# mrjoshuak/go-jpeg2000

Measured on AMD Instinct MI355X. Metric: Mpixels/s encode+decode (4K sRGB, 5-3 lossless), higher is better.
Workload: dtype int32

## Files before the change

go-jpeg2000_amd/csrc/ht.hip:

```cpp
#include <cstdlib>

#include "ht_tables.h"
#include "j2k_internal.h"

namespace j2k {

__device__ __constant__ uint16_t c_vlc_tbl0[1024] = J2K_HT_VLC_TBL0_INIT;
__device__ __constant__ uint16_t c_vlc_tbl1[1024] = J2K_HT_VLC_TBL1_INIT;
__device__ uint16_t g_vlc_enc[2 * 4 * 16];

__global__ void ht_build_enc_table() {
    const int t = threadIdx.x;
    if (t >= 128) return;
    const int initial = t >> 6, context = (t >> 4) & 3, rho = t & 15;
    const uint16_t *tbl = initial ? c_vlc_tbl0 : c_vlc_tbl1;
    uint16_t r = 0x0001;
    for (uint32_t cwd = 0; cwd < 128; cwd++) {
        const uint16_t e = tbl[(context << 7) | cwd];
        if (((e >> 4) & 0xF) == rho && (e & 0xF) > 0) { r = (uint16_t)((cwd << 4) | (e & 0xF)); break; }
    }
    g_vlc_enc[t] = r;
}

__device__ uint16_t g_vlc_pair1[16384];
// ... 1126 lines not shown
                                                         const uint32_t *__restrict__ lens, uint32_t *__restrict__ vbits,
                                                         uint32_t *__restrict__ pairs) {
    __shared__ uint32_t vb4[4][HT_VBITS_WORDS + 8];
    uint32_t *vb = vb4[threadIdx.x >> 6];
    const int jid = blockIdx.x * 4 + (threadIdx.x >> 6);
    if (jid >= njobs) return;
    const int lane = threadIdx.x & 63;
    if (ht_vlcprep_block(jobs, jid, stream, offs, lens, lane, vb, pairs + (size_t)jid * HT_WALK_REC)) return;
    uint32_t *dst = vbits + (size_t)jid * HT_VBITS_WORDS;
    for (int i = lane; i < HT_VBITS_WORDS; i += 64) dst[i] = vb[i];
}

__global__ __launch_bounds__(256) void ht_vlcprep_dedup_kernel(const BlockJob *__restrict__ jobs, int njobs,
                                                               const uint8_t *__restrict__ stream, const uint64_t *__restrict__ offs,
                                                               const uint32_t *__restrict__ lens, uint32_t *__restrict__ vbits,
                                                               uint32_t *__restrict__ pairs, const int32_t *__restrict__ rep) {
    __shared__ uint32_t vb4[4][HT_VBITS_WORDS + 8];
    uint32_t *vb = vb4[threadIdx.x >> 6];
    const int jid = blockIdx.x * 4 + (threadIdx.x >> 6);
    if (jid >= njobs) return;
    const int lane = threadIdx.x & 63;
    uint32_t *rec = pairs + (size_t)jid * HT_WALK_REC;
    const int ldr = rep[jid];
    const uint64_t loff = offs[ldr];
    const uint32_t llen = lens[ldr];
    const HtVlcHead H = ht_vlc_head(jobs, jid, stream, offs, lens);
    const long nb = H.tag ? 0 : ht_vlc_nbytes(H);
    uint32_t pre[HT_VLC_STEPS];
#pragma unroll
    for (int c = 0; c < HT_VLC_STEPS; c++) pre[c] = ht_vlc_load4(H.data, (long)H.len, nb, 1 + 256 * c + 4 * lane);
    if (ldr != jid && H.tag == 0 && llen == H.len && H.len >= 4) {
        const uint8_t *mine = H.data, *theirs = stream + loff;
        const uint32_t len = H.len, nd = (len + 3) >> 2;
        bool same = true;
        for (uint32_t j0 = 0; j0 < nd && same; j0 += 256) {
            uint32_t x[4], y[4];
#pragma unroll
            for (int c = 0; c < 4; c++) {
                const uint32_t p = min(4 * (j0 + 64 * c + lane), len - 4);
                __builtin_memcpy(&x[c], mine + p, 4);
                __builtin_memcpy(&y[c], theirs + p, 4);
            }
            same = __all((x[0] == y[0]) & (x[1] == y[1]) & (x[2] == y[2]) & (x[3] == y[3]));
        }
        if (same) {
            if (lane == 0) { rec[0] = HT_PAIR_DUP; rec[1] = (uint32_t)ldr; rec[HT_WALK_MAX_PAIRS] = H.scup; }
            return;
        }
    }
    ht_vlc_unstuff(H, lane, vb, rec, pre);
    if (H.tag) return;
    uint32_t *dst = vbits + (size_t)jid * HT_VBITS_WORDS;
    for (int i = lane; i < HT_VBITS_WORDS; i += 64) dst[i] = vb[i];
}

#ifndef HT_WALK_BLOCKS
#define HT_WALK_BLOCKS 64
#endif
struct HtWalkShared {
    uint32_t vb[HT_WALK_BLOCKS][HT_VROW];
    uint16_t pair1[16384];
    uint16_t tbl0[512], tbl1[512];
};

__device__ __forceinline__ uint32_t uvlc_used_later(uint32_t vlc, uint32_t uOff1, uint32_t uOff2) {
    const uint32_t t1 = uOff2 ? uvlc_entry(vlc) : 0u;
    const uint32_t pl1 = t1 & 3;
// ... 47 lines not shown
            const uint32_t vw = __builtin_amdgcn_alignbit(w1, w0, len);
            const uint32_t m1 = (uint32_t)((int32_t)(e << 18) >> 31), m2 = (uint32_t)((int32_t)(e << 17) >> 31);
            const uint32_t pl1 = (0x12131213u >> ((vw & 7) << 2)) & 3 & m1;
            const uint32_t t1 = (0x12141218u >> ((vw & 7) << 2)) & 0xF & m1;
            const uint32_t t2 = (0x12141218u >> (((vw >> pl1) & 7) << 2)) & 0xF & m2;
            pos += len + t1 + t2;
            rec[it] = (e & 0x7FFF) | vw << 16;
        }
    }
#undef HT_FETCH
    return pos;
}

template <bool DEDUP>
__global__ __launch_bounds__(256) void ht_walk_kernel(const BlockJob *__restrict__ jobs, int njobs,
                                                     const uint32_t *__restrict__ vbits, uint32_t *__restrict__ pairs) {
    extern __shared__ __align__(16) unsigned char walk_smem[];
    HtWalkShared &S = *reinterpret_cast<HtWalkShared *>(walk_smem);
    const int tid = threadIdx.x, lane = tid & 63;
    const int jid0 = blockIdx.x * HT_WALK_BLOCKS;
    const int jid = jid0 + lane;
    const bool have = lane < HT_WALK_BLOCKS && jid < njobs;
#ifdef J2K_WALK_STAMP
    const long long st0 = __builtin_amdgcn_s_memtime();
#endif
    const int nblk = min(HT_WALK_BLOCKS, njobs - jid0);
    uint32_t *rec = pairs + (size_t)jid * HT_WALK_REC;
    uint32_t tag = HT_PAIR_ZERO;
    int w = 0, h = 0;
    if (tid < 64 && have) { tag = rec[0]; w = jobs[jid].w; h = jobs[jid].h; }
    {
        constexpr int NV = HT_WALK_BLOCKS * 48 / 256;
        uint4 t[8], v[NV];
#pragma unroll
        for (int j = 0; j < 8; j++) t[j] = reinterpret_cast<const uint4 *>(g_vlc_pair1)[j * 256 + tid];
#pragma unroll
        for (int j = 0; j < NV; j++) {
            const int q = j * 256 + tid;
            const int bsel = min(q / 48, nblk - 1);
            v[j] = reinterpret_cast<const uint4 *>(vbits + (size_t)(jid0 + bsel) * HT_VBITS_WORDS)[q % 48];
        }
        if (tid < 64) reinterpret_cast<uint4 *>(S.tbl0)[tid] = reinterpret_cast<const uint4 *>(c_vlc_tbl0)[tid];
        else if (tid < 128) reinterpret_cast<uint4 *>(S.tbl1)[tid - 64] = reinterpret_cast<const uint4 *>(c_vlc_tbl1)[tid - 64];
#pragma unroll
        for (int j = 0; j < 8; j++) reinterpret_cast<uint4 *>(S.pair1)[j * 256 + tid] = t[j];
#pragma unroll
        for (int j = 0; j < NV; j++) {
            const int q = j * 256 + tid;
            uint32_t *d = &S.vb[q / 48][4 * (q % 48)];
            d[0] = v[j].x; d[1] = v[j].y; d[2] = v[j].z; d[3] = v[j].w;
        }
    }
    __syncthreads();
#ifdef J2K_WALK_STAMP
    const long long st1 = __builtin_amdgcn_s_memtime();
#endif
    if (tid >= 64) return;
    const uint32_t pos = ht_walk_lane<DEDUP>(&S.vb[lane][0], S.tbl0, S.tbl1, S.pair1, rec, w, h, have, tag);
    (void)pos;
#ifdef J2K_WALK_STAMP
    const long long st2 = __builtin_amdgcn_s_memtime();
    if ((blockIdx.x == 0 || blockIdx.x == 50) && lane == 0)
        printf("walk wg %d: staging %lld cyc, loop %lld cyc (%d x %d, %d bits)\n", (int)blockIdx.x, st1 - st0, st2 - st1, w, h, (int)pos);
#endif
}

#ifndef HT_FRONT_NW
#define HT_FRONT_NW 16
#endif
#ifndef HT_FRONT_PRIO
#define HT_FRONT_PRIO 0
#endif
// ... 796 lines not shown
                                   uint64_t *offs, uint32_t *lens, uint8_t *numbps, uint64_t *status, uint32_t epoch, int *fault) {
    if (njobs <= 0) return hipSuccess;
    hipError_t e;
    if ((e = ht_tables_ready(s)) != hipSuccess) return e;
    hipLaunchKernelGGL(ht_encode_stream_kernel, dim3(njobs), dim3(64), 0, s, jobs, njobs, coef, stream,
                       reinterpret_cast<unsigned long long *>(offs), lens, numbps, reinterpret_cast<unsigned long long *>(status), epoch, fault);
    return hipGetLastError();
}
int ht_fast_max_samples() { return HT_FAST_MAX_SAMPLES; }
int ht_walk_max_pairs() { return HT_WALK_MAX_PAIRS; }

size_t ht_decode_scratch_words(int njobs) { return (size_t)njobs * (HT_WALK_REC + HT_VBITS_WORDS); }

hipError_t launch_ht_decode(hipStream_t s, const BlockJob *jobs, int njobs, const uint8_t *stream, const uint64_t *offs,
                            const uint32_t *lens, int32_t *decoded, uint32_t *scratch, int coded_rows_only, const BlockJob *placed_jobs, int lean,
                            int front, const int32_t *dedup_rep, const int32_t *dedup_fol) {
    const bool dedup = dedup_rep && dedup_fol && !placed_jobs && lean && front != 1;
    if (njobs <= 0) return hipSuccess;
    hipError_t e;
    if ((e = ht_tables_ready(s)) != hipSuccess) return e;
    uint32_t *pairs = scratch, *vbits = scratch + (size_t)njobs * HT_WALK_REC;
    if (front == 1) {
        for (int rep_ = 0; rep_ < dev_reps(32 | 64); rep_++)
        hipLaunchKernelGGL(ht_front_kernel<HT_FRONT_NW>, dim3((njobs + HT_WALK_BLOCKS - 1) / HT_WALK_BLOCKS), dim3(64 * HT_FRONT_NW), sizeof(HtFrontShared), s, jobs, njobs, stream, offs, lens, pairs);
    } else {
        for (int rep_ = 0; rep_ < dev_reps(32); rep_++)
        if (dedup) hipLaunchKernelGGL(ht_vlcprep_dedup_kernel, dim3((njobs + 3) / 4), dim3(256), 0, s, jobs, njobs, stream, offs, lens, vbits, pairs, dedup_rep);
        else
        hipLaunchKernelGGL(ht_vlcprep_kernel, dim3((njobs + 3) / 4), dim3(256), 0, s, jobs, njobs, stream, offs, lens, vbits, pairs);
        if ((e = hipGetLastError()) != hipSuccess) return e;
        for (int rep_ = 0; rep_ < dev_reps(64); rep_++)
        if (dedup) hipLaunchKernelGGL(ht_walk_kernel<true>, dim3((njobs + HT_WALK_BLOCKS - 1) / HT_WALK_BLOCKS), dim3(256), sizeof(HtWalkShared), s, jobs, njobs, vbits, pairs);
        else
        hipLaunchKernelGGL(ht_walk_kernel<false>, dim3((njobs + HT_WALK_BLOCKS - 1) / HT_WALK_BLOCKS), dim3(256), sizeof(HtWalkShared), s, jobs, njobs, vbits, pairs);
    }
    if ((e = hipGetLastError()) != hipSuccess) return e;
    for (int rep_ = 0; rep_ < dev_reps(128); rep_++)
    if (dedup) hipLaunchKernelGGL((ht_decode_lean_kernel<false, true>), dim3((njobs + 3) / 4), dim3(256), 0, s, jobs, njobs, stream, offs, lens, decoded, pairs, coded_rows_only, dedup_fol);
    else if (placed_jobs) {
        if (lean) hipLaunchKernelGGL((ht_decode_lean_kernel<true, false>), dim3((njobs + 3) / 4), dim3(256), 0, s, placed_jobs, njobs, stream, offs, lens, decoded, pairs, 1, (const int32_t *)nullptr);
        else hipLaunchKernelGGL(ht_decode_kernel<true>, dim3((njobs + 3) / 4), dim3(256), 0, s, placed_jobs, njobs, stream, offs, lens, decoded, pairs, 1);
    }
    else
    if (lean) hipLaunchKernelGGL((ht_decode_lean_kernel<false, false>), dim3((njobs + 3) / 4), dim3(256), 0, s, jobs, njobs, stream, offs, lens, decoded, pairs, coded_rows_only, (const int32_t *)nullptr);
    else hipLaunchKernelGGL(ht_decode_kernel<false>, dim3((njobs + 3) / 4), dim3(256), 0, s, jobs, njobs, stream, offs, lens, decoded, pairs, coded_rows_only);
    return hipGetLastError();
}

}
// ... 1 lines not shown
```

go-jpeg2000_amd/csrc/j2k_frame.cpp:

```cpp
#include "j2k_host.h"

using namespace j2k;

extern "C" int j2k_t2_encode_packets_device(j2k_ctx *ctx, const j2k_t2_dev_packet *d_packets, size_t npackets, const j2k_t2_dev_cb *d_cbs, size_t ncbs,
                                            const uint8_t *d_data, int sop, int eph, uint8_t *bio_delay, uint8_t *d_out, size_t cap,
                                            uint64_t *d_offs, size_t *total) {
    if (!ctx || !bio_delay || !d_offs || !total || (npackets && !d_packets) || (ncbs && !d_cbs) || (cap && !d_out)) return J2K_ERR_INVALID_ARG;
    if (ctx->capturing) return fail(ctx, J2K_ERR_INVALID_ARG, "a synchronising call while the context captures a graph");
    if (npackets > ((size_t)1 << 31)) return fail(ctx, J2K_ERR_INVALID_ARG, "too many packets");
    HIPCHK(ctx, hipSetDevice(ctx->device));
    const size_t ws = j2k::t2_dev_workspace((long)npackets);
    int r = stage_reserve(ctx, 1, ws + 64);
    if (r != J2K_OK) return r;
    uint64_t *d_res = reinterpret_cast<uint64_t *>((uint8_t *)ctx->stage[1] + ((ws + 15) & ~size_t(15)));
    HIPCHK(ctx, hipMemsetAsync(d_res, 0, 3 * sizeof(uint64_t), ctx->stream));
    HIPCHK(ctx, j2k::launch_t2_encode_packets(ctx->stream, d_packets, (long)npackets, d_cbs, (uint64_t)ncbs, d_data, sop, eph, *bio_delay ? 1 : 0, d_out, (uint64_t)cap,
                                              d_offs, ctx->stage[1], d_res));
    uint64_t res[3] = {0, 0, 0};
    HIPCHK(ctx, hipMemcpyAsync(res, d_res, sizeof(res), hipMemcpyDeviceToHost, ctx->stream));
    HIPCHK(ctx, hipStreamSynchronize(ctx->stream));
    if (res[2]) return fail(ctx, J2K_ERR_GO_PANIC, "packet coder: a tag tree of width 0 (the reference divides by it, t2.go:328,348), or a packet whose code-blocks lie outside the table");
    *total = (size_t)res[0];
    if (res[0] > cap) return fail(ctx, J2K_ERR_CAPACITY, "packet coder: the output buffer is smaller than the packets");
    *bio_delay = res[1] ? 1 : 0;
// ... 430 lines not shown

extern "C" int j2k_plan_get_decoded_offsets(const j2k_plan *P, uint64_t *offs, size_t cap) {
    if (!P || !offs) return J2K_ERR_INVALID_ARG;
    if (cap < P->dec_off.size()) return J2K_ERR_CAPACITY;
    if (!P->dec_off.empty()) memcpy(offs, P->dec_off.data(), P->dec_off.size() * sizeof(uint64_t));
    return J2K_OK;
}

extern "C" int j2k_plan_get_ht_decode_leaders(const j2k_plan *P, int32_t *leaders, size_t cap) {
    if (!P || !leaders) return J2K_ERR_INVALID_ARG;
    if (P->spec.coder != J2K_CODER_HT) return J2K_ERR_UNSUPPORTED;
    if (cap < P->ht_dec_rep.size()) return J2K_ERR_CAPACITY;
    if (!P->ht_dec_rep.empty()) memcpy(leaders, P->ht_dec_rep.data(), P->ht_dec_rep.size() * sizeof(int32_t));
    return J2K_OK;
}
```

go-jpeg2000_amd/csrc/j2k_host.h:

```cpp
#pragma once
#include <algorithm>
#include <atomic>
#include <cstdio>
#include <cstdlib>
#include <cstring>
#include <map>
#include <tuple>

#include "j2k_plan.h"

namespace j2k {
#ifdef J2K_DEV
int g_dev_skip = 0, g_dev_dup = 0;
#endif
hipError_t launch_add_const(hipStream_t s, int32_t *d, size_t n, int delta);
hipError_t launch_rct(hipStream_t s, int32_t *a, int32_t *b, int32_t *c, size_t n, int inverse);
hipError_t launch_ict(hipStream_t s, double *a, double *b, double *c, size_t n, int inverse);
hipError_t launch_dwt97_fwd(hipStream_t s, const LevelLaunch &L, const void *src, int src_is_f64, int32_t *out_i32,
                            double *out_f64, double *nxt, int dc_shift, int quant, double step, int mct);
hipError_t launch_dwt97_inv(hipStream_t s, const LevelLaunch &L, const void *coef, int coef_is_f64, const double *prev,
                            void *dst, int dc_shift, int final_level, int dst_mode, int mct, double step);
hipError_t launch_quantize97(hipStream_t s, const double *src, size_t n, double step, int32_t *dst);
hipError_t launch_dequantize97(hipStream_t s, const int32_t *src, size_t n, double step, double *dst);
hipError_t launch_ht_encode(hipStream_t s, const BlockJob *jobs, int njobs, const int32_t *coef, uint8_t *slots,
                            uint32_t *lens, uint8_t *numbps, int *fault, uint32_t *maglens = nullptr, const HtUJob *utab = nullptr, int nunique = 0,
                            const int *alias_ids = nullptr, int waves = 1);
hipError_t launch_ht_decode(hipStream_t s, const BlockJob *jobs, int njobs, const uint8_t *stream, const uint64_t *offs,
                            const uint32_t *lens, int32_t *decoded, uint32_t *scratch, int coded_rows_only = 0, const BlockJob *placed_jobs = nullptr, int lean = 1, int front = 3,
                            const int32_t *dedup_rep = nullptr, const int32_t *dedup_fol = nullptr);
int ht_walk_max_pairs();
size_t ht_decode_scratch_words(int njobs);
hipError_t launch_ht_encode_stream(hipStream_t s, const BlockJob *jobs, int njobs, const int32_t *coef, uint8_t *stream,
                                   uint64_t *offs, uint32_t *lens, uint8_t *numbps, uint64_t *status, uint32_t epoch, int *fault);
int ht_fast_max_samples();
hipError_t launch_t1_encode(hipStream_t s, const BlockJob *jobs, int njobs, const int32_t *coef, uint8_t *slots,
                            uint32_t *lens, uint8_t *numbps, uint8_t *work, size_t work_per_job, int *fault, int max_dim,
                            uint8_t *sym, size_t sym_stride, uint32_t *nsyms, int lanes, uint8_t *bigsym = nullptr, const uint64_t *bigsym_off = nullptr,
                            uint32_t *bignsyms = nullptr, uint32_t *rate = nullptr);
hipError_t launch_rate_distortion(hipStream_t s, const BlockJob *jobs, int njobs, const int32_t *coef, const uint8_t *numbps, uint64_t *dist);
hipError_t launch_roi_windows(hipStream_t s, const j2k_block *blocks, int n, const AreaPlane *planes, int x0, int y0, int x1, int y1, int margin, int32_t *win);
hipError_t launch_rate_distortion_roi(hipStream_t s, const BlockJob *jobs, int njobs, const int32_t *coef, const uint8_t *numbps, const j2k_block *blocks,
                                      const AreaPlane *planes, int x0, int y0, int x1, int y1, int margin, uint32_t gain, uint64_t *dist);
size_t rate_allocate_workspace(int njobs);
hipError_t launch_rate_allocate(hipStream_t s, int njobs, const uint32_t *rate, const uint64_t *dist, const uint8_t *numbps, const double *weights,
// ... 123 lines not shown
```

go-jpeg2000_amd/csrc/j2k_plan.h:

```cpp
#pragma once
#include <string>
#include <vector>

#include "../../include/j2kgfx.h"
#include "j2k_internal.h"

struct j2k_ctx {
    int device = -1;
    hipStream_t stream = nullptr;
    std::string last_error;
    int fuse_compact = 0;
    int fwd_link = 1;
    int inv_link = 1;
    int pix_fuse = 1;
    bool plane_wg3 = false;
    int plane_wg = 4;
    int l0_fuse = 0;
    int l0_wg = 8;
    int l0_wg_invw = 4;
    bool l0_deal = true;
    int l0_wg97 = 8;
    int plane_wg97 = 8;
    int l0_wg97_inv = 8;
    int l0_xcd_group = 16;
// ... 170 lines not shown
    std::vector<uint64_t> dec_off;
    j2k::BlockJob *d_bjobs = nullptr;
    j2k::BlockJob *d_djobs = nullptr;
    j2k::BlockJob *d_djobs_placed = nullptr;
    int64_t bytes_cap = 0, decoded_elems = 0, block_samples = 0;
    int64_t dwt_bytes = 0, dwt_level0_bytes = 0;
    void *d_frame = nullptr, *d_coeff = nullptr, *d_slots = nullptr, *d_stream = nullptr;
    void *d_lens = nullptr, *d_numbps = nullptr, *d_offs = nullptr;
    j2k::DwtJob *d_fwd_pix_jobs = nullptr;
    int fwd_pix_njobs = 0;
    j2k::HtUJob *d_ht_ujobs = nullptr; int *d_ht_alias_next = nullptr;
    j2k::BlockJob *d_bjobs_alias = nullptr;
    int ht_nunique = 0;
    std::vector<int32_t> ht_dec_rep;
    int32_t *d_ht_dec_rep = nullptr, *d_ht_dec_fol = nullptr;
    j2k::DwtJob *d_fwd97_wg_jobs = nullptr;
    int fwd97_wg_njobs = 0, fwd97_wg_waves = 0;
    j2k::DwtJob *d_inv97_wg_jobs = nullptr;
    int inv97_wg_njobs = 0, inv97_wg_waves = 0;
    j2k::DwtJob *d_fwd_wg2_jobs = nullptr, *d_fwd_wg_rest_jobs = nullptr;
    int fwd_wg2_njobs = 0, fwd_wg2_waves = 0, fwd_wg_rest_njobs = 0;
    j2k::DwtJob *d_fwd_wg_jobs = nullptr;
    int fwd_wg_njobs = 0, fwd_wg_waves = 0;
    j2k::DwtJob *d_inv_wg_jobs = nullptr;
    int inv_wg_njobs = 0, inv_wg_waves = 0;
    uint32_t *d_maglens = nullptr;
    uint32_t *d_mels = nullptr;
    const void *last_stream = nullptr, *last_lens = nullptr;
    bool want_toffs = false, toffs_valid = false;
    uint64_t *d_toffs = nullptr;
// ... 22 lines not shown
```

go-jpeg2000_amd/csrc/j2k_planbuild.cpp:

```cpp
#include "j2k_host.h"

using namespace j2k;

bool PlanSpec::operator==(const PlanSpec &o) const {
    return W == o.W && H == o.H && C == o.C && tile_w == o.tile_w && tile_h == o.tile_h && levels == o.levels &&
           frame_h == o.frame_h && wavelet == o.wavelet && precision == o.precision && dc_shift == o.dc_shift && dc_shift_inv == o.dc_shift_inv && mct == o.mct && quant == o.quant && quality == o.quality &&
           num_res_jobs == o.num_res_jobs && cb_w == o.cb_w && cb_h == o.cb_h && coder == o.coder &&
           tile_first == o.tile_first && tile_count == o.tile_count && frame_is_f64 == o.frame_is_f64 && closed_loop == o.closed_loop && mallat == o.mallat;
}

static inline int pick_cpl(int maxw) { return maxw >= 384 ? 8 : (maxw >= 192 ? 4 : 2); }

struct LevelRule { int cpl; bool vec; int halo; };
static LevelRule level_rule(const PlanSpec &S, int cls, const std::vector<DwtPlane> &planes, int maxw, int frame_stride, int cpl0, bool vec_ok) {
    int cpl = pick_cpl(maxw);
    if (cpl0 > 0 && S.wavelet == W53) cpl = cpl0;
    if (S.wavelet == W97) cpl = (cls == 1) ? 2 : (maxw >= 192 ? 4 : 2);
    for (size_t i = 0; i < planes.size() && vec_ok; i++) {
        const DwtPlane &D = planes[i];
        if (D.w % cpl) vec_ok = false;
        if (frame_stride > 0 && (frame_stride % cpl)) vec_ok = false;
        for (int k = 0; k < 3; k++)
            if ((D.src_off[k] % 4) || (D.out_off[k] % 4) || (D.nxt_off[k] % 4)) vec_ok = false;
    }
// ... 609 lines not shown
            bool any = false;
            for (size_t i = 0; i < nj; i++) {
                P->ht_dec_rep[i] = (int32_t)i;
                auto ins = lead.emplace(std::make_tuple(bj[i].src_off, bj[i].stride, bj[i].w, bj[i].h), (int)i);
                if (ins.second) continue;
                const int L = ins.first->second, w = bj[i].w, h = bj[i].h;
                const int R = (h + 3) / 4, Np = R * (((w + 3) / 4 + 1) / 2);
                const bool fast = (size_t)R * (size_t)w <= (size_t)ht_fast_max_samples() && Np <= ht_walk_max_pairs();
                int32_t *row = &fol[(size_t)L * (J2K_HT_DEC_MAX_FOLLOWERS + 1)];
                if (bj[L].w != w || bj[L].h != h || !(w == 8 || w == 16 || w == 32 || w == 64) || !fast) continue;
                if ((P->dec_off[i] & 3) || (P->dec_off[L] & 3) || row[0] >= J2K_HT_DEC_MAX_FOLLOWERS) continue;
                row[++row[0]] = (int32_t)i;
                P->ht_dec_rep[i] = L;
                any = true;
            }
            if (any) {
                r = upload(ctx, &P->d_ht_dec_rep, P->ht_dec_rep);
                if (r == J2K_OK) r = upload(ctx, &P->d_ht_dec_fol, fol);
            }
        }
        for (size_t i = 0; i < bj.size(); i++) bj[i].out_off = (int64_t)P->dec_off[i];
        if (r == J2K_OK) r = upload(ctx, &P->d_djobs, bj);
        if (r == J2K_OK && P->spec.closed_loop && P->spec.coder == J2K_CODER_HT) {
            for (size_t i = 0; i < bj.size(); i++) bj[i].out_off = bj[i].src_off;
            r = upload(ctx, &P->d_djobs_placed, bj);
        }
        if (r != J2K_OK) { j2k_plan_destroy(P); return r; }
    }
    *out = P;
    return J2K_OK;
}

static void free_reduced(ReducedTab &R) {
// ... 122 lines not shown
    *width = (int32_t)(((int64_t)S.W + m) >> reduce);
    *height = (int32_t)(((int64_t)S.H + m) >> reduce);
    return J2K_OK;
}

extern "C" void j2k_plan_destroy(j2k_plan *P) {
    if (!P) return;
    if (P->ctx) { (void)hipSetDevice(P->ctx->device); (void)hipStreamSynchronize(P->ctx->stream); }
    for (ReducedTab &R : P->reduced) free_reduced(R);
    free_layer_tabs(P);
    for (int cls = 0; cls < 2; cls++) {
        for (auto &T : P->fwd[cls]) { if (T.d_planes) (void)hipFree(T.d_planes); if (T.d_jobs) (void)hipFree(T.d_jobs); if (T.d_pjobs) (void)hipFree(T.d_pjobs); }
        if (cls == 0 && P->d_bigsym_off) { (void)hipFree(P->d_bigsym_off); P->d_bigsym_off = nullptr; }
        for (auto &T : P->inv[cls]) { if (T.d_planes) (void)hipFree(T.d_planes); if (T.d_jobs) (void)hipFree(T.d_jobs); if (T.d_pjobs) (void)hipFree(T.d_pjobs); }
    }
    void *ptrs[] = {P->d_deep_jobs_inv, P->d_mega_fwd_jobs, P->d_mega_inv_jobs, P->d_fwd_top_jobs, P->d_inv_top_jobs, P->d_inv_wg_jobs, P->d_deep_planes, P->d_deep_jobs, P->d_tile_job0, P->d_scrA, P->d_scrB, P->d_tail, P->d_bjobs, P->d_djobs, P->d_djobs_placed, P->d_frame, P->d_coeff, P->d_slots, P->d_stream, P->d_lens, P->d_numbps, P->d_offs, P->d_status, P->d_fwd_pix_jobs, P->d_fwd_wg2_jobs, P->d_fwd_wg_rest_jobs, P->d_fwd_wg_jobs, P->d_fwd97_wg_jobs, P->d_inv97_wg_jobs, P->d_ht_ujobs, P->d_ht_alias_next, P->d_ht_dec_rep, P->d_ht_dec_fol, P->d_bjobs_alias, P->d_maglens, P->d_mels, P->d_toffs,
                    P->d_t2_packets, P->d_tile_packet0, P->d_t2_cbs, P->d_t2_poffs, P->d_t2_ptile, P->d_t2_ws, P->d_t2_chains, P->d_t2_body_base, P->d_t2_par, P->d_frame_status,
                    P->d_cl_decoded, P->d_cl_coeff, P->d_cl_coeff_dec, P->d_cl_numbps, P->d_cl_offs, P->d_cl_lens, P->d_host_io, P->d_host_pix,
                    P->d_rate_wj, P->d_rate_ws, P->d_cl_rate, P->d_cl_dense, P->d_cl_lfloors,
                    P->d_area_blocks, P->d_area_planes, P->d_area_frame};
    for (void *p : ptrs) if (p) (void)hipFree(p);
    delete P;
}

static int spec_from_params(j2k_ctx *ctx, const j2k_params *p, PlanSpec &S) {
    if (!p) return fail(ctx, J2K_ERR_INVALID_ARG, "params == NULL");
    if (p->precision < 1 || p->precision > 31) return fail(ctx, J2K_ERR_INVALID_ARG, "precision out of range");
    S.W = p->width; S.H = p->height; S.C = p->ncomp;
    S.frame_h = p->frame_rows > 0 ? p->frame_rows : p->height;
    if (S.frame_h > 0 && p->height % S.frame_h) return fail(ctx, J2K_ERR_INVALID_ARG, "height is not a whole number of frames (frame_rows)");
    S.tile_w = p->tile_w; S.tile_h = p->tile_h;
// ... 57 lines not shown
```

go-jpeg2000_amd/csrc/j2k_stages.cpp:

```cpp
#include "j2k_host.h"

using namespace j2k;

static LevelLaunch mk(const LevelTab &T, int pf = 0) {
    LevelLaunch L{T.d_jobs, T.njobs, T.d_planes, T.cpl, T.vec, T.ncomp, pf};
    L.pjobs = T.d_pjobs; L.pnjobs = T.p_pix_only ? 0 : T.pnjobs; L.pwaves = T.pwaves; L.pmulti = T.pmulti;
    L.mallat = T.mallat ? 1 : 0;
    return L;
}

static void pix_launch(LevelLaunch &L, const LevelTab &T, const PixIO &pix, int cls, const PlanSpec &S) {
    L.pix_stride = pix.stride;
    L.pix_src = cls ? (pix.triple == 4 ? 4 : 0) : pix.single;
    L.comp_elems = (long long)S.W * S.H;
    if (cls == 1 && pix.triple == 4) L.pnjobs = T.pnjobs;
}

int plan_forward_impl(j2k_plan *P, const void *d_frame, void *d_coeff, PixIO pix) {
    const int pix_stride = pix.stride;
    j2k_ctx *ctx = P->ctx;
    const PlanSpec &S = P->spec;
    if (((uintptr_t)d_frame & 15) || ((uintptr_t)d_coeff & 15)) return fail(ctx, J2K_ERR_INVALID_ARG, "device pointers must be 16-byte aligned");
    HIPCHK(ctx, hipSetDevice(ctx->device));
    const double step = 1.0 / (double)S.quality;
// ... 815 lines not shown
    const int r = check_skip_planes(P->ctx, P->spec.coder, skip_planes, "j2k_plan_decode_blocks_floors");
    if (r != J2K_OK) return r;
    if (d_floors && P->spec.coder == J2K_CODER_HT) return fail(P->ctx, J2K_ERR_UNSUPPORTED, "j2k_plan_decode_blocks_floors: per-block floors need the MQ coder");
    return plan_decode_blocks_jobs(P, P->d_djobs, (int)P->blocks.size(), d_stream, d_offs, d_lens, d_numbps, d_decoded, nullptr, skip_planes, d_floors);
}

int plan_decode_blocks_jobs(j2k_plan *P, const BlockJob *d_djobs, int n, const uint8_t *d_stream, const uint64_t *d_offs, const uint32_t *d_lens,
                            const uint8_t *d_numbps, int32_t *d_decoded, const BlockJob *d_placed, int skip_planes, const uint8_t *d_floors) {
    j2k_ctx *ctx = P->ctx;
    HIPCHK(ctx, hipSetDevice(ctx->device));
    if (!n) return J2K_OK;
    if (P->spec.coder == J2K_CODER_HT) {
        int r = stage_reserve(ctx, 2, ht_decode_scratch_words(n) * 4 + 256);
        if (r != J2K_OK) return r;
        const bool dedup = ctx->ht_dec_dedup && d_djobs == P->d_djobs && n == (int)P->blocks.size() && !d_placed && ctx->ht_dec_lean == 1 &&
                           ctx->ht_dec_front == 3 && P->d_ht_dec_rep && P->d_ht_dec_fol;
        HIPCHK(ctx, launch_ht_decode(ctx->stream, d_djobs, n, d_stream, d_offs, d_lens, d_decoded, (uint32_t *)ctx->stage[2],
                                     (d_placed || P->dec_coded_rows_only) ? 1 : 0, d_placed, ctx->ht_dec_lean, ctx->ht_dec_front,
                                     dedup ? P->d_ht_dec_rep : nullptr, dedup ? P->d_ht_dec_fol : nullptr));
    } else {
        size_t wpj = 0;
        int max_dim = 0;
        for (const j2k_block &b : P->blocks) { wpj = std::max(wpj, t1_flag_bytes(b.w, b.h)); max_dim = std::max(max_dim, std::max(b.w, b.h)); }
        wpj = (wpj + 255) & ~size_t(255);
        const int split_min = ctx->t1_dec_split >= 0 ? ctx->t1_dec_split : (mq_throughput_mode() ? 512 : 12000);
        bool split = split_min > 0 && n >= split_min && !ctx->t1_dec_general && !((uintptr_t)d_stream & 15);
        const size_t gen_bytes = (wpj * (size_t)n + 255) & ~size_t(255);
        int r = stage_reserve(ctx, 2, gen_bytes + 256 + (split ? j2k::t1_dec_split_bytes((size_t)n) : 0));
        if (r != J2K_OK && split) { (void)hipGetLastError(); split = false; r = stage_reserve(ctx, 2, gen_bytes + 256); }
        if (r != J2K_OK) return r;
        HIPCHK(ctx, launch_t1_decode(ctx->stream, d_djobs, n, d_stream, d_offs, d_lens, d_numbps, d_decoded,
                                     (uint8_t *)ctx->stage[2], wpj, max_dim, ctx->t1_dec_general,
                                     split ? (uint8_t *)ctx->stage[2] + gen_bytes : nullptr, ctx->t1_dec_lanes, mq_throughput_mode() ? 1 : 0, skip_planes, d_floors));
    }
// ... 4 lines not shown
```

go-jpeg2000_amd/j2kgfx/_lib.py:

```python
import ctypes as C
import os

_PKG = os.path.dirname(os.path.abspath(__file__))
LIB_PATH = os.environ.get("J2K_LIB") or os.path.join(os.path.dirname(_PKG), "libj2kgfx.so")

OK = 0
ERR_INVALID_ARG, ERR_NO_DEVICE, ERR_HIP, ERR_CAPACITY, ERR_GO_PANIC, ERR_UNSUPPORTED = -1, -2, -3, -4, -5, -6
BAND_LL, BAND_HL, BAND_LH, BAND_HH = 0, 1, 2, 3
CODER_MQ, CODER_HT = 0, 1


class J2KError(RuntimeError):
    def __init__(self, status, msg=""):
        self.status = status
        super().__init__("j2kgfx status %d: %s" % (status, msg))


class Block(C.Structure):
    _fields_ = [("plane", C.c_int32), ("band", C.c_int32), ("x0", C.c_int32), ("y0", C.c_int32),
                ("w", C.c_int32), ("h", C.c_int32)]


class Params(C.Structure):
    _fields_ = [(n, C.c_int32) for n in (
# ... 9 lines not shown

SYMBOLS = [
    "j2k_ctx_create", "j2k_ctx_destroy", "j2k_ctx_sync", "j2k_ctx_stream", "j2k_ctx_last_error",
    "j2k_status_string", "j2k_version", "j2k_ctx_set_option", "j2k_ctx_profile_enable", "j2k_ctx_profile_read", "j2k_ctx_profile_read_tag",
    "j2k_ctx_capture_begin", "j2k_ctx_capture_end", "j2k_graph_launch", "j2k_graph_destroy",
    "j2k_dc_level_shift_forward", "j2k_dc_level_shift_inverse", "j2k_forward_rct", "j2k_inverse_rct",
    "j2k_forward_ict", "j2k_inverse_ict",
    "j2k_forward53", "j2k_inverse53", "j2k_forward97", "j2k_inverse97",
    "j2k_forward2d53", "j2k_inverse2d53", "j2k_forward2d97", "j2k_inverse2d97",
    "j2k_decompose_multilevel53", "j2k_reconstruct_multilevel53",
    "j2k_decompose_multilevel97", "j2k_reconstruct_multilevel97",
    "j2k_tcd_apply_forward_dwt", "j2k_tcd_apply_inverse_dwt", "j2k_quantize", "j2k_dequantize",
    "j2k_encode_blocks", "j2k_decode_blocks", "j2k_block_bound",
    "j2k_plan_set_decode_coded_rows_only", "j2k_plan_set_dequantize", "j2k_plan_create", "j2k_plan_destroy", "j2k_plan_get_info", "j2k_plan_get_blocks", "j2k_plan_get_planes",
    "j2k_plan_forward", "j2k_plan_inverse", "j2k_plan_encode_blocks", "j2k_plan_compact", "j2k_plan_encode_stream",
    "j2k_plan_decode_blocks", "j2k_plan_get_decoded_offsets", "j2k_plan_get_ht_decode_leaders", "j2k_encode_frame",
    "j2k_mq_encode", "j2k_mq_decode", "j2k_raw_encode", "j2k_raw_decode",
    "j2k_convert_colorspace", "j2k_convert_colorspace_device",
    "j2k_pixels_components", "j2k_pixels_precision", "j2k_extract_image_data", "j2k_create_image",
    "j2k_unpack_pixels", "j2k_pack_pixels", "j2k_plan_forward_rgba8", "j2k_plan_inverse_rgba8",
    "j2k_plan_forward_pixels", "j2k_plan_inverse_pixels", "j2k_plan_pixels_fused",
    "j2k_image_validate", "j2k_image_to_rgba8", "j2k_extract_image_planar", "j2k_plan_forward_image", "j2k_plan_image_fused",
    "j2k_plan_encode_frame_image", "j2k_encode_image_host",
    "j2k_tile_part_bound", "j2k_create_tile_header", "j2k_assemble_tiles", "j2k_read_tile_part_header", "j2k_parse_tile_parts",
    "j2k_plan_tile_parts_bound", "j2k_plan_assemble_tiles_device",
    "j2k_t2_packet_sequence", "j2k_t2_packet_bound", "j2k_t2_encode_packet", "j2k_t2_decode_packet", "j2k_t2_encode_packets_device", "j2k_t2_decode_packets_device", "j2k_plan_t2_packets", "j2k_plan_t2_fill_cbs", "j2k_tagtree_shape", "j2k_tcd_init_tile",
    "j2k_plan_frame_bound", "j2k_plan_encode_tile_parts", "j2k_plan_decode_tile_parts", "j2k_plan_place_blocks", "j2k_plan_frame_status", "j2k_plan_frame_parallel_tiles",
    "j2k_plan_encode_frame_pixels", "j2k_plan_decode_frame_pixels", "j2k_encode_pixels_host", "j2k_decode_pixels_host",
    "j2k_plan_reduced_size", "j2k_plan_inverse_reduced", "j2k_plan_inverse_pixels_reduced", "j2k_plan_decode_frame_pixels_reduced", "j2k_decode_pixels_host_reduced",
    "j2k_decode_blocks_coarse", "j2k_plan_decode_blocks_coarse", "j2k_plan_decode_frame_pixels_coarse", "j2k_decode_pixels_host_coarse",
    "j2k_decode_blocks_floors", "j2k_plan_decode_blocks_floors",
# ... 109 lines not shown
```

go-jpeg2000_amd/j2kgfx/codec.py:

```python
import functools
import ctypes as C
import sys

import numpy as np

from . import _lib
from .context import default_context

BLOCK_DTYPE = np.dtype([("plane", "<i4"), ("band", "<i4"), ("x0", "<i4"), ("y0", "<i4"), ("w", "<i4"), ("h", "<i4")])


def _torch():
    import torch
    return torch


def _stage(fn):
    @functools.wraps(fn)
    def wrapped(self, *a, **k):
        if self.track_streams:
            t = _torch()
            self._ext().wait_stream(t.cuda.current_stream(self.device))
        return fn(self, *a, **k)
    return wrapped
# ... 53 lines not shown
        out = np.zeros((n, 7), dtype=np.int64)
        self.ctx.check(self.ctx.L.j2k_plan_get_planes(self.h, out.ctypes.data_as(C.c_void_p), C.c_size_t(n)))
        return out

    def decoded_offsets(self):
        n = int(self.info.blocks)
        out = np.zeros(max(n, 1), dtype=np.uint64)
        self.ctx.check(self.ctx.L.j2k_plan_get_decoded_offsets(self.h, out.ctypes.data_as(C.c_void_p), C.c_size_t(n)))
        return out[:n]

    def ht_decode_leaders(self):
        n = int(self.info.blocks)
        out = np.zeros(max(n, 1), dtype=np.int32)
        self.ctx.check(self.ctx.L.j2k_plan_get_ht_decode_leaders(self.h, out.ctypes.data_as(C.c_void_p), C.c_size_t(n)))
        return out[:n]

    def empty(self, n, dtype):
        t = _torch()
        return t.empty(max(int(n), 4), dtype=dtype, device=self.device)

    def alloc_coeff(self):
        return self.empty(self.info.coeff_elems, _torch().int32)

    def alloc_frame(self):
        t = _torch()
        return t.empty((self.ncomp, self.height, self.width), dtype=t.int32, device=self.device)

    def _ext(self):
        if self._ext_stream is None:
            self._ext_stream = _torch().cuda.ExternalStream(self.ctx.stream, device=self.device)
# ... 641 lines not shown
```

include/j2kgfx.h:

```cpp
#ifndef J2KGFX_H
#define J2KGFX_H

#include <stddef.h>
#include <stdint.h>

#ifdef __cplusplus
extern "C" {
#endif

#define J2K_OK 0
#define J2K_ERR_INVALID_ARG (-1)
#define J2K_ERR_NO_DEVICE (-2)
#define J2K_ERR_HIP (-3)
#define J2K_ERR_CAPACITY (-4)
#define J2K_ERR_GO_PANIC (-5)
#define J2K_ERR_UNSUPPORTED (-6)

#define J2K_BAND_LL 0
#define J2K_BAND_HL 1
#define J2K_BAND_LH 2
#define J2K_BAND_HH 3

#define J2K_CODER_MQ 0
#define J2K_CODER_HT 1
// ... 110 lines not shown
int j2k_plan_encode_stream(j2k_plan *plan, const int32_t *d_coeff, uint8_t *d_stream, uint64_t *d_offs,
                           uint32_t *d_lens, uint8_t *d_numbps);
size_t j2k_plan_pack_bound(const j2k_plan *plan);
int j2k_plan_pack_stream(j2k_plan *plan, const uint8_t *d_stream, const uint64_t *d_offs, const uint32_t *d_lens,
                         const uint8_t *d_numbps, uint8_t *d_pack);
int j2k_plan_unpack_stream(j2k_plan *plan, const uint8_t *d_pack, size_t pack_bytes, uint8_t *d_stream, uint64_t *d_offs,
                           uint32_t *d_lens, uint8_t *d_numbps);
int j2k_plan_unpack_streams(j2k_plan *plan, int count, const uint8_t *const *d_packs, const size_t *pack_bytes,
                            uint8_t *const *d_streams, uint64_t *const *d_offs, uint32_t *const *d_lens, uint8_t *const *d_numbps);
int j2k_plan_decode_blocks(j2k_plan *plan, const uint8_t *d_stream, const uint64_t *d_offs,
                           const uint32_t *d_lens, const uint8_t *d_numbps, int32_t *d_decoded);
int j2k_plan_set_decode_coded_rows_only(j2k_plan *plan, int on);
int j2k_plan_set_dequantize(j2k_plan *plan, int on);
int j2k_plan_get_decoded_offsets(const j2k_plan *plan, uint64_t *offs, size_t cap);
int j2k_plan_get_ht_decode_leaders(const j2k_plan *plan, int32_t *leaders, size_t cap);

typedef struct j2k_comm j2k_comm;
#define J2K_COMM_ID_BYTES 128
#define J2K_GATHER_SELF_LOOP 1
const char *j2k_comm_load_error(void);
int j2k_comm_get_unique_id(uint8_t *id128);
int j2k_comm_create(j2k_ctx *ctx, const uint8_t *id128, int rank, int world, j2k_comm **out);
void j2k_comm_destroy(j2k_comm *comm);
const char *j2k_comm_last_error(j2k_comm *comm);
void *j2k_comm_stream(j2k_comm *comm);
int j2k_gather_streams(j2k_comm *comm, int count, const uint8_t *const *d_send, const uint64_t *send_bytes,
                       const uint64_t *all_bytes, j2k_ctx *const *producers, int nproducers,
                       uint8_t *d_recv, size_t recv_cap, uint64_t *recv_offs, int flags);
int j2k_comm_wait(j2k_comm *comm, j2k_ctx *consumer);

// ... 242 lines not shown
```

Before: 82370.

## Reorder HT decode walk to pack leader blocks first and skip follower-only workgroups

The plan builder now computes a walk order that places dedup leader codeblocks first and followers after, plus an inverse position map. The vlcprep dedup kernel writes unstuffed VLC bits into the reordered slot and shortens the byte comparison against the leader by reusing already-loaded prefix words and comparing only up to the MEL/VLC boundary plus the tail. The walk kernel reads jobs through the order array, so workgroups made entirely of duplicate or zero followers can exit early instead of loading tables and walking. This adds an indirection and a tag probe per workgroup, and relies on the shortened comparison being enough to prove the streams are identical.

```diff
diff --git a/go-jpeg2000_amd/csrc/ht.hip b/go-jpeg2000_amd/csrc/ht.hip
--- a/go-jpeg2000_amd/csrc/ht.hip
+++ b/go-jpeg2000_amd/csrc/ht.hip
@@ -1164,7 +1164,8 @@
 __global__ __launch_bounds__(256) void ht_vlcprep_dedup_kernel(const BlockJob *__restrict__ jobs, int njobs,
                                                                const uint8_t *__restrict__ stream, const uint64_t *__restrict__ offs,
                                                                const uint32_t *__restrict__ lens, uint32_t *__restrict__ vbits,
-                                                               uint32_t *__restrict__ pairs, const int32_t *__restrict__ rep) {
+                                                               uint32_t *__restrict__ pairs, const int32_t *__restrict__ rep,
+                                                               const int32_t *__restrict__ walk_pos) {
     __shared__ uint32_t vb4[4][HT_VBITS_WORDS + 8];
     uint32_t *vb = vb4[threadIdx.x >> 6];
     const int jid = blockIdx.x * 4 + (threadIdx.x >> 6);
@@ -1172,6 +1173,7 @@
     const int lane = threadIdx.x & 63;
     uint32_t *rec = pairs + (size_t)jid * HT_WALK_REC;
     const int ldr = rep[jid];
+    const int slot = walk_pos[jid];
     const uint64_t loff = offs[ldr];
     const uint32_t llen = lens[ldr];
     const HtVlcHead H = ht_vlc_head(jobs, jid, stream, offs, lens);
@@ -1181,13 +1183,29 @@
     for (int c = 0; c < HT_VLC_STEPS; c++) pre[c] = ht_vlc_load4(H.data, (long)H.len, nb, 1 + 256 * c + 4 * lane);
     if (ldr != jid && H.tag == 0 && llen == H.len && H.len >= 4) {
         const uint8_t *mine = H.data, *theirs = stream + loff;
-        const uint32_t len = H.len, nd = (len + 3) >> 2;
-        bool same = true;
-        for (uint32_t j0 = 0; j0 < nd && same; j0 += 256) {
-            uint32_t x[4], y[4];
+        const uint32_t len = H.len;
+        uint32_t aend = min(len, len - H.scup + 4);
+        if (aend >= len - 2 - (uint32_t)nb) aend = len;
+        const uint32_t nd = (aend + 3) >> 2;
+        uint32_t x[4], y[4], lb[HT_VLC_STEPS], tx, ty;
+#pragma unroll
+        for (int c = 0; c < HT_VLC_STEPS; c++) lb[c] = ht_vlc_load4(theirs, (long)len, nb, 1 + 256 * c + 4 * lane);
+        __builtin_memcpy(&tx, mine + (len - 4), 4);
+        __builtin_memcpy(&ty, theirs + (len - 4), 4);
+#pragma unroll
+        for (int c = 0; c < 4; c++) {
+            const uint32_t p = min(4 * (64 * c + lane), aend - 4);
+            __builtin_memcpy(&x[c], mine + p, 4);
+            __builtin_memcpy(&y[c], theirs + p, 4);
+        }
+        bool eq = tx == ty;
+#pragma unroll
+        for (int c = 0; c < HT_VLC_STEPS; c++) eq &= pre[c] == lb[c];
+        bool same = __all(eq & (x[0] == y[0]) & (x[1] == y[1]) & (x[2] == y[2]) & (x[3] == y[3]));
+        for (uint32_t j0 = 256; j0 < nd && same; j0 += 256) {
 #pragma unroll
             for (int c = 0; c < 4; c++) {
-                const uint32_t p = min(4 * (j0 + 64 * c + lane), len - 4);
+                const uint32_t p = min(4 * (j0 + 64 * c + lane), aend - 4);
                 __builtin_memcpy(&x[c], mine + p, 4);
                 __builtin_memcpy(&y[c], theirs + p, 4);
             }
@@ -1200,7 +1218,7 @@
     }
     ht_vlc_unstuff(H, lane, vb, rec, pre);
     if (H.tag) return;
-    uint32_t *dst = vbits + (size_t)jid * HT_VBITS_WORDS;
+    uint32_t *dst = vbits + (size_t)slot * HT_VBITS_WORDS;
     for (int i = lane; i < HT_VBITS_WORDS; i += 64) dst[i] = vb[i];
 }
 
@@ -1278,20 +1296,31 @@
 
 template <bool DEDUP>
 __global__ __launch_bounds__(256) void ht_walk_kernel(const BlockJob *__restrict__ jobs, int njobs,
-                                                     const uint32_t *__restrict__ vbits, uint32_t *__restrict__ pairs) {
+                                                     const uint32_t *__restrict__ vbits, uint32_t *__restrict__ pairs,
+                                                     const int32_t *__restrict__ walk_order, int nlead) {
     extern __shared__ __align__(16) unsigned char walk_smem[];
     HtWalkShared &S = *reinterpret_cast<HtWalkShared *>(walk_smem);
     const int tid = threadIdx.x, lane = tid & 63;
     const int jid0 = blockIdx.x * HT_WALK_BLOCKS;
-    const int jid = jid0 + lane;
-    const bool have = lane < HT_WALK_BLOCKS && jid < njobs;
+    const bool have = lane < HT_WALK_BLOCKS && jid0 + lane < njobs;
+    int jid = jid0 + lane;
+    if constexpr (DEDUP) {
+        jid = walk_order[min(jid0 + lane, njobs - 1)];
+        if (jid0 >= nlead) {
+            int fj = jid;
+            asm volatile("" : "+v"(fj));
+            const uint32_t t = pairs[(size_t)fj * HT_WALK_REC];
+            if (!__any(have && t != HT_PAIR_SERIAL && t != HT_PAIR_ZERO && t != HT_PAIR_DUP)) return;
+        }
+    }
 #ifdef J2K_WALK_STAMP
     const long long st0 = __builtin_amdgcn_s_memtime();
 #endif
     const int nblk = min(HT_WALK_BLOCKS, njobs - jid0);
-    uint32_t *rec = pairs + (size_t)jid * HT_WALK_REC;
+    uint32_t *rec = DEDUP ? nullptr : pairs + (size_t)jid * HT_WALK_REC;
     uint32_t tag = HT_PAIR_ZERO;
     int w = 0, h = 0;
+    if constexpr (!DEDUP)
     if (tid < 64 && have) { tag = rec[0]; w = jobs[jid].w; h = jobs[jid].h; }
     {
         constexpr int NV = HT_WALK_BLOCKS * 48 / 256;
@@ -1304,6 +1333,10 @@
             const int bsel = min(q / 48, nblk - 1);
             v[j] = reinterpret_cast<const uint4 *>(vbits + (size_t)(jid0 + bsel) * HT_VBITS_WORDS)[q % 48];
         }
+        if constexpr (DEDUP) {
+            rec = pairs + (size_t)jid * HT_WALK_REC;
+            tag = rec[0]; w = jobs[jid].w; h = jobs[jid].h;
+        }
         if (tid < 64) reinterpret_cast<uint4 *>(S.tbl0)[tid] = reinterpret_cast<const uint4 *>(c_vlc_tbl0)[tid];
         else if (tid < 128) reinterpret_cast<uint4 *>(S.tbl1)[tid - 64] = reinterpret_cast<const uint4 *>(c_vlc_tbl1)[tid - 64];
 #pragma unroll
@@ -1320,6 +1353,9 @@
     const long long st1 = __builtin_amdgcn_s_memtime();
 #endif
     if (tid >= 64) return;
+    if constexpr (DEDUP) {
+        if (!have) { tag = HT_PAIR_ZERO; w = 0; h = 0; }
+    }
     const uint32_t pos = ht_walk_lane<DEDUP>(&S.vb[lane][0], S.tbl0, S.tbl1, S.pair1, rec, w, h, have, tag);
     (void)pos;
 #ifdef J2K_WALK_STAMP
@@ -2146,8 +2182,8 @@
 
 hipError_t launch_ht_decode(hipStream_t s, const BlockJob *jobs, int njobs, const uint8_t *stream, const uint64_t *offs,
                             const uint32_t *lens, int32_t *decoded, uint32_t *scratch, int coded_rows_only, const BlockJob *placed_jobs, int lean,
-                            int front, const int32_t *dedup_rep, const int32_t *dedup_fol) {
-    const bool dedup = dedup_rep && dedup_fol && !placed_jobs && lean && front != 1;
+                            int front, const int32_t *dedup_rep, const int32_t *dedup_fol, const int32_t *walk_order, const int32_t *walk_pos, int walk_nlead) {
+    const bool dedup = dedup_rep && dedup_fol && walk_order && walk_pos && !placed_jobs && lean && front != 1;
     if (njobs <= 0) return hipSuccess;
     hipError_t e;
     if ((e = ht_tables_ready(s)) != hipSuccess) return e;
@@ -2157,14 +2193,14 @@
         hipLaunchKernelGGL(ht_front_kernel<HT_FRONT_NW>, dim3((njobs + HT_WALK_BLOCKS - 1) / HT_WALK_BLOCKS), dim3(64 * HT_FRONT_NW), sizeof(HtFrontShared), s, jobs, njobs, stream, offs, lens, pairs);
     } else {
         for (int rep_ = 0; rep_ < dev_reps(32); rep_++)
-        if (dedup) hipLaunchKernelGGL(ht_vlcprep_dedup_kernel, dim3((njobs + 3) / 4), dim3(256), 0, s, jobs, njobs, stream, offs, lens, vbits, pairs, dedup_rep);
+        if (dedup) hipLaunchKernelGGL(ht_vlcprep_dedup_kernel, dim3((njobs + 3) / 4), dim3(256), 0, s, jobs, njobs, stream, offs, lens, vbits, pairs, dedup_rep, walk_pos);
         else
         hipLaunchKernelGGL(ht_vlcprep_kernel, dim3((njobs + 3) / 4), dim3(256), 0, s, jobs, njobs, stream, offs, lens, vbits, pairs);
         if ((e = hipGetLastError()) != hipSuccess) return e;
         for (int rep_ = 0; rep_ < dev_reps(64); rep_++)
-        if (dedup) hipLaunchKernelGGL(ht_walk_kernel<true>, dim3((njobs + HT_WALK_BLOCKS - 1) / HT_WALK_BLOCKS), dim3(256), sizeof(HtWalkShared), s, jobs, njobs, vbits, pairs);
+        if (dedup) hipLaunchKernelGGL(ht_walk_kernel<true>, dim3((njobs + HT_WALK_BLOCKS - 1) / HT_WALK_BLOCKS), dim3(256), sizeof(HtWalkShared), s, jobs, njobs, vbits, pairs, walk_order, walk_nlead);
         else
-        hipLaunchKernelGGL(ht_walk_kernel<false>, dim3((njobs + HT_WALK_BLOCKS - 1) / HT_WALK_BLOCKS), dim3(256), sizeof(HtWalkShared), s, jobs, njobs, vbits, pairs);
+        hipLaunchKernelGGL(ht_walk_kernel<false>, dim3((njobs + HT_WALK_BLOCKS - 1) / HT_WALK_BLOCKS), dim3(256), sizeof(HtWalkShared), s, jobs, njobs, vbits, pairs, (const int32_t *)nullptr, 0);
     }
     if ((e = hipGetLastError()) != hipSuccess) return e;
     for (int rep_ = 0; rep_ < dev_reps(128); rep_++)
diff --git a/go-jpeg2000_amd/csrc/j2k_frame.cpp b/go-jpeg2000_amd/csrc/j2k_frame.cpp
--- a/go-jpeg2000_amd/csrc/j2k_frame.cpp
+++ b/go-jpeg2000_amd/csrc/j2k_frame.cpp
@@ -468,3 +468,12 @@
     if (!P->ht_dec_rep.empty()) memcpy(leaders, P->ht_dec_rep.data(), P->ht_dec_rep.size() * sizeof(int32_t));
     return J2K_OK;
 }
+
+extern "C" int j2k_plan_get_ht_decode_walk_order(const j2k_plan *P, int32_t *order, size_t cap, int32_t *n_leaders) {
+    if (!P || !order) return J2K_ERR_INVALID_ARG;
+    if (P->spec.coder != J2K_CODER_HT) return J2K_ERR_UNSUPPORTED;
+    if (cap < P->ht_walk_order.size()) return J2K_ERR_CAPACITY;
+    if (!P->ht_walk_order.empty()) memcpy(order, P->ht_walk_order.data(), P->ht_walk_order.size() * sizeof(int32_t));
+    if (n_leaders) *n_leaders = (int32_t)P->ht_walk_nlead;
+    return J2K_OK;
+}
diff --git a/go-jpeg2000_amd/csrc/j2k_host.h b/go-jpeg2000_amd/csrc/j2k_host.h
--- a/go-jpeg2000_amd/csrc/j2k_host.h
+++ b/go-jpeg2000_amd/csrc/j2k_host.h
@@ -27,7 +27,8 @@
                             const int *alias_ids = nullptr, int waves = 1);
 hipError_t launch_ht_decode(hipStream_t s, const BlockJob *jobs, int njobs, const uint8_t *stream, const uint64_t *offs,
                             const uint32_t *lens, int32_t *decoded, uint32_t *scratch, int coded_rows_only = 0, const BlockJob *placed_jobs = nullptr, int lean = 1, int front = 3,
-                            const int32_t *dedup_rep = nullptr, const int32_t *dedup_fol = nullptr);
+                            const int32_t *dedup_rep = nullptr, const int32_t *dedup_fol = nullptr, const int32_t *walk_order = nullptr,
+                            const int32_t *walk_pos = nullptr, int walk_nlead = 0);
 int ht_walk_max_pairs();
 size_t ht_decode_scratch_words(int njobs);
 hipError_t launch_ht_encode_stream(hipStream_t s, const BlockJob *jobs, int njobs, const int32_t *coef, uint8_t *stream,
diff --git a/go-jpeg2000_amd/csrc/j2k_plan.h b/go-jpeg2000_amd/csrc/j2k_plan.h
--- a/go-jpeg2000_amd/csrc/j2k_plan.h
+++ b/go-jpeg2000_amd/csrc/j2k_plan.h
@@ -208,6 +208,9 @@
     int ht_nunique = 0;
     std::vector<int32_t> ht_dec_rep;
     int32_t *d_ht_dec_rep = nullptr, *d_ht_dec_fol = nullptr;
+    std::vector<int32_t> ht_walk_order;
+    int32_t *d_ht_walk_order = nullptr, *d_ht_walk_pos = nullptr;
+    int ht_walk_nlead = 0;
     j2k::DwtJob *d_fwd97_wg_jobs = nullptr;
     int fwd97_wg_njobs = 0, fwd97_wg_waves = 0;
     j2k::DwtJob *d_inv97_wg_jobs = nullptr;
diff --git a/go-jpeg2000_amd/csrc/j2k_planbuild.cpp b/go-jpeg2000_amd/csrc/j2k_planbuild.cpp
--- a/go-jpeg2000_amd/csrc/j2k_planbuild.cpp
+++ b/go-jpeg2000_amd/csrc/j2k_planbuild.cpp
@@ -647,9 +647,17 @@
                 P->ht_dec_rep[i] = L;
                 any = true;
             }
+            P->ht_walk_order.clear();
+            for (size_t i = 0; i < nj; i++) if (P->ht_dec_rep[i] == (int32_t)i) P->ht_walk_order.push_back((int32_t)i);
+            P->ht_walk_nlead = (int)P->ht_walk_order.size();
+            for (size_t i = 0; i < nj; i++) if (P->ht_dec_rep[i] != (int32_t)i) P->ht_walk_order.push_back((int32_t)i);
             if (any) {
+                std::vector<int32_t> pos(nj);
+                for (size_t s = 0; s < nj; s++) pos[(size_t)P->ht_walk_order[s]] = (int32_t)s;
                 r = upload(ctx, &P->d_ht_dec_rep, P->ht_dec_rep);
                 if (r == J2K_OK) r = upload(ctx, &P->d_ht_dec_fol, fol);
+                if (r == J2K_OK) r = upload(ctx, &P->d_ht_walk_order, P->ht_walk_order);
+                if (r == J2K_OK) r = upload(ctx, &P->d_ht_walk_pos, pos);
             }
         }
         for (size_t i = 0; i < bj.size(); i++) bj[i].out_off = (int64_t)P->dec_off[i];
@@ -802,7 +810,7 @@
         if (cls == 0 && P->d_bigsym_off) { (void)hipFree(P->d_bigsym_off); P->d_bigsym_off = nullptr; }
         for (auto &T : P->inv[cls]) { if (T.d_planes) (void)hipFree(T.d_planes); if (T.d_jobs) (void)hipFree(T.d_jobs); if (T.d_pjobs) (void)hipFree(T.d_pjobs); }
     }
-    void *ptrs[] = {P->d_deep_jobs_inv, P->d_mega_fwd_jobs, P->d_mega_inv_jobs, P->d_fwd_top_jobs, P->d_inv_top_jobs, P->d_inv_wg_jobs, P->d_deep_planes, P->d_deep_jobs, P->d_tile_job0, P->d_scrA, P->d_scrB, P->d_tail, P->d_bjobs, P->d_djobs, P->d_djobs_placed, P->d_frame, P->d_coeff, P->d_slots, P->d_stream, P->d_lens, P->d_numbps, P->d_offs, P->d_status, P->d_fwd_pix_jobs, P->d_fwd_wg2_jobs, P->d_fwd_wg_rest_jobs, P->d_fwd_wg_jobs, P->d_fwd97_wg_jobs, P->d_inv97_wg_jobs, P->d_ht_ujobs, P->d_ht_alias_next, P->d_ht_dec_rep, P->d_ht_dec_fol, P->d_bjobs_alias, P->d_maglens, P->d_mels, P->d_toffs,
+    void *ptrs[] = {P->d_deep_jobs_inv, P->d_mega_fwd_jobs, P->d_mega_inv_jobs, P->d_fwd_top_jobs, P->d_inv_top_jobs, P->d_inv_wg_jobs, P->d_deep_planes, P->d_deep_jobs, P->d_tile_job0, P->d_scrA, P->d_scrB, P->d_tail, P->d_bjobs, P->d_djobs, P->d_djobs_placed, P->d_frame, P->d_coeff, P->d_slots, P->d_stream, P->d_lens, P->d_numbps, P->d_offs, P->d_status, P->d_fwd_pix_jobs, P->d_fwd_wg2_jobs, P->d_fwd_wg_rest_jobs, P->d_fwd_wg_jobs, P->d_fwd97_wg_jobs, P->d_inv97_wg_jobs, P->d_ht_ujobs, P->d_ht_alias_next, P->d_ht_dec_rep, P->d_ht_dec_fol, P->d_ht_walk_order, P->d_ht_walk_pos, P->d_bjobs_alias, P->d_maglens, P->d_mels, P->d_toffs,
                     P->d_t2_packets, P->d_tile_packet0, P->d_t2_cbs, P->d_t2_poffs, P->d_t2_ptile, P->d_t2_ws, P->d_t2_chains, P->d_t2_body_base, P->d_t2_par, P->d_frame_status,
                     P->d_cl_decoded, P->d_cl_coeff, P->d_cl_coeff_dec, P->d_cl_numbps, P->d_cl_offs, P->d_cl_lens, P->d_host_io, P->d_host_pix,
                     P->d_rate_wj, P->d_rate_ws, P->d_cl_rate, P->d_cl_dense, P->d_cl_lfloors,
diff --git a/go-jpeg2000_amd/csrc/j2k_stages.cpp b/go-jpeg2000_amd/csrc/j2k_stages.cpp
--- a/go-jpeg2000_amd/csrc/j2k_stages.cpp
+++ b/go-jpeg2000_amd/csrc/j2k_stages.cpp
@@ -853,10 +853,11 @@
         int r = stage_reserve(ctx, 2, ht_decode_scratch_words(n) * 4 + 256);
         if (r != J2K_OK) return r;
         const bool dedup = ctx->ht_dec_dedup && d_djobs == P->d_djobs && n == (int)P->blocks.size() && !d_placed && ctx->ht_dec_lean == 1 &&
-                           ctx->ht_dec_front == 3 && P->d_ht_dec_rep && P->d_ht_dec_fol;
+                           ctx->ht_dec_front == 3 && P->d_ht_dec_rep && P->d_ht_dec_fol && P->d_ht_walk_order && P->d_ht_walk_pos;
         HIPCHK(ctx, launch_ht_decode(ctx->stream, d_djobs, n, d_stream, d_offs, d_lens, d_decoded, (uint32_t *)ctx->stage[2],
                                      (d_placed || P->dec_coded_rows_only) ? 1 : 0, d_placed, ctx->ht_dec_lean, ctx->ht_dec_front,
-                                     dedup ? P->d_ht_dec_rep : nullptr, dedup ? P->d_ht_dec_fol : nullptr));
+                                     dedup ? P->d_ht_dec_rep : nullptr, dedup ? P->d_ht_dec_fol : nullptr, dedup ? P->d_ht_walk_order : nullptr,
+                                     dedup ? P->d_ht_walk_pos : nullptr, dedup ? P->ht_walk_nlead : 0));
     } else {
         size_t wpj = 0;
         int max_dim = 0;
diff --git a/go-jpeg2000_amd/j2kgfx/_lib.py b/go-jpeg2000_amd/j2kgfx/_lib.py
--- a/go-jpeg2000_amd/j2kgfx/_lib.py
+++ b/go-jpeg2000_amd/j2kgfx/_lib.py
@@ -47,7 +47,7 @@
     "j2k_encode_blocks", "j2k_decode_blocks", "j2k_block_bound",
     "j2k_plan_set_decode_coded_rows_only", "j2k_plan_set_dequantize", "j2k_plan_create", "j2k_plan_destroy", "j2k_plan_get_info", "j2k_plan_get_blocks", "j2k_plan_get_planes",
     "j2k_plan_forward", "j2k_plan_inverse", "j2k_plan_encode_blocks", "j2k_plan_compact", "j2k_plan_encode_stream",
-    "j2k_plan_decode_blocks", "j2k_plan_get_decoded_offsets", "j2k_plan_get_ht_decode_leaders", "j2k_encode_frame",
+    "j2k_plan_decode_blocks", "j2k_plan_get_decoded_offsets", "j2k_plan_get_ht_decode_leaders", "j2k_plan_get_ht_decode_walk_order", "j2k_encode_frame",
     "j2k_mq_encode", "j2k_mq_decode", "j2k_raw_encode", "j2k_raw_decode",
     "j2k_convert_colorspace", "j2k_convert_colorspace_device",
     "j2k_pixels_components", "j2k_pixels_precision", "j2k_extract_image_data", "j2k_create_image",
diff --git a/go-jpeg2000_amd/j2kgfx/codec.py b/go-jpeg2000_amd/j2kgfx/codec.py
--- a/go-jpeg2000_amd/j2kgfx/codec.py
+++ b/go-jpeg2000_amd/j2kgfx/codec.py
@@ -91,6 +91,13 @@
         out = np.zeros(max(n, 1), dtype=np.int32)
         self.ctx.check(self.ctx.L.j2k_plan_get_ht_decode_leaders(self.h, out.ctypes.data_as(C.c_void_p), C.c_size_t(n)))
         return out[:n]
+
+    def ht_decode_walk_order(self):
+        n = int(self.info.blocks)
+        out = np.zeros(max(n, 1), dtype=np.int32)
+        nl = C.c_int32(0)
+        self.ctx.check(self.ctx.L.j2k_plan_get_ht_decode_walk_order(self.h, out.ctypes.data_as(C.c_void_p), C.c_size_t(n), C.byref(nl)))
+        return out[:n], int(nl.value)
 
     def empty(self, n, dtype):
         t = _torch()
diff --git a/include/j2kgfx.h b/include/j2kgfx.h
--- a/include/j2kgfx.h
+++ b/include/j2kgfx.h
@@ -148,6 +148,7 @@
 int j2k_plan_set_dequantize(j2k_plan *plan, int on);
 int j2k_plan_get_decoded_offsets(const j2k_plan *plan, uint64_t *offs, size_t cap);
 int j2k_plan_get_ht_decode_leaders(const j2k_plan *plan, int32_t *leaders, size_t cap);
+int j2k_plan_get_ht_decode_walk_order(const j2k_plan *plan, int32_t *order, size_t cap, int32_t *n_leaders);
 
 typedef struct j2k_comm j2k_comm;
 #define J2K_COMM_ID_BYTES 128
```

Result: no change. 83630 (median of 6 runs) (+1.5%).
